# ghnmqdtg/VM-ASR

Hardware: AMD Instinct MI355X
Metric: audio clips/sec (train step) 48kHz n_fft=1024 (higher is better)
Workload: dtype bf16 (autocast over G; scan/STFT f32; MPD f32/bf16x3 MFMA); 1 GPU; vm_asr_48k_MPD.yaml full train step, DIMS 16 d_state 1 n_fft 1024 clip 122640@48k; per_gpu_batch=4, global_batch=4, parallelism=dp1, execution=hipGraph replay, 2 streams, generator_streams=2

## Files before the change

### include/vmasr_hip.h

```cpp
#ifndef VMASR_HIP_H
#define VMASR_HIP_H

#include <stddef.h>
#include <stdint.h>

#ifdef __cplusplus
extern "C" {
#endif

#define VMASR_ABI_VERSION 1

typedef void *vmasr_stream_t;

enum { VMASR_F32 = 0, VMASR_F16 = 1, VMASR_BF16 = 2 };

enum {
    VMASR_OK = 0,
    VMASR_EINVAL = -1,
    VMASR_EALIGN = -2,
    VMASR_ENOSPACE = -3
};

int vmasr_abi_version(void);
const char *vmasr_last_error(void);
// ... 181 lines not shown
    const float *bias;
    int64_t nseq;
    int32_t H;
    int32_t reserved;
} vmasr_cg_slot;
int vmasr_conv_mfma_supported(int32_t Cin, int32_t Cout, int32_t k, int32_t stride);
int vmasr_conv_mfma_supported_launch(int32_t Cin, int32_t Cout, int32_t k, int32_t stride, int32_t n, int64_t rows);
int vmasr_conv_mfma_config(int32_t pass, int32_t Cin, int32_t Cout, int32_t ops, int32_t out[3]);
void vmasr_conv_set_cu_limit(int32_t cus);
int32_t vmasr_conv_get_cu_limit(void);
int vmasr_conv_mfma_fwd(const vmasr_cg_slot *slots, int32_t n, int32_t Cin, int32_t Cout, int32_t k, int32_t stride, int32_t pad,
                        int64_t rows_out, int32_t act, vmasr_stream_t stream);
int vmasr_conv_mfma_dgrad(const vmasr_cg_slot *slots, int32_t n, int32_t Cin, int32_t Cout, int32_t k, int32_t stride, int32_t pad,
                          int64_t rows_in, vmasr_stream_t stream);
int vmasr_conv_f32_fwd(const vmasr_cg_slot *slots, int32_t n, int32_t Cin, int32_t Cout, int32_t k, int32_t stride, int32_t pad,
                       int64_t rows_out, int32_t act, vmasr_stream_t stream);
int vmasr_conv_f32_dgrad(const vmasr_cg_slot *slots, int32_t n, int32_t Cin, int32_t Cout, int32_t k, int32_t stride, int32_t pad,
                         int64_t rows_in, vmasr_stream_t stream);
int vmasr_conv_mfma_wgrad(const vmasr_cg_slot *slots, int32_t n, int32_t Cin, int32_t Cout, int32_t k, int32_t stride, int32_t pad,
                          int32_t splits, vmasr_stream_t stream);
typedef struct vmasr_cg_gelu_bwd {
    const float *pre;
    const signed char *sgn;
    int64_t valid;
    float scale;
    int32_t reserved;
    float *db;
} vmasr_cg_gelu_bwd;
int vmasr_conv_mfma_dgrad_gelu(const vmasr_cg_slot *slots, const vmasr_cg_gelu_bwd *epi, const float *gtok, int32_t n, int32_t Cin, int32_t Cout,
                               int32_t k, int32_t stride, int32_t pad, int64_t rows_in, vmasr_stream_t stream);

int vmasr_wgrad_finish_multi(const float *const *parts, float *const *dws, float *const *dbs, float *const *e1s, float *const *e2s,
                             const int32_t *Ss, const int32_t *Ns, const int32_t *Ks, const int32_t *lds, int32_t n, vmasr_stream_t stream);

int vmasr_linear_f64acc(const float *x, const float *w, const float *bias, float *y, int64_t rows, int32_t out_features,
                        int32_t in_features, vmasr_stream_t stream);

typedef struct vmasr_adamw_item {
    float *p;
    const float *g;
    float *m;
    float *v;
    void *lp;
    int64_t n;
    float weight_decay;
    int32_t vec;
    void *lpt;
    int32_t rows, cols;
} vmasr_adamw_item;
int32_t vmasr_adamw_chunk(void);
int vmasr_adamw_step(const vmasr_adamw_item *items, const int32_t *chunks, int32_t nchunks, int64_t total_elems, const float *lr,
                     const float *step, float beta1, float beta2, float eps, vmasr_stream_t stream);

typedef struct vmasr_grad_segment {
    const float *ptr;
    int64_t n;
} vmasr_grad_segment;
size_t vmasr_grad_norm_workspace(int32_t nchunks);
int vmasr_grad_norm(const vmasr_grad_segment *segments, const int32_t *chunks, int32_t nchunks, int64_t total_elems, float max_norm,
                    float *state, void *workspace, size_t ws_bytes, vmasr_stream_t stream);
int vmasr_adamw_step_guarded(const vmasr_adamw_item *items, const int32_t *chunks, int32_t nchunks, int64_t total_elems, const float *lr,
                             const float *step, float beta1, float beta2, float eps, const float *state, float *const *step_counters,
                             int32_t ncounters, vmasr_stream_t stream);

typedef struct vmasr_sgd_item {
    float *p;
// ... 221 lines not shown
    VMASR_K_BIAS_GELU,
    VMASR_K_SS2D_TRANSPOSE,
    VMASR_K_SS2D_FWD_AGG,
    VMASR_K_SS2D_CARRY,
    VMASR_K_SS2D_FWD_APPLY,
    VMASR_K_SS2D_MERGE,
    VMASR_K_SS2D_BWD_AGG,
    VMASR_K_SS2D_BWD_APPLY,
    VMASR_K_SS2D_PRE,
    VMASR_K_LN_GATE,
    VMASR_K_STACK_ROWS,
    VMASR_K_FEAT_L1,
    VMASR_K_ADAMW,
    VMASR_K_CONV_POST,
    VMASR_K_CONV_POST_BWD_GELU,
    VMASR_K_WEIGHT_T,
    VMASR_K_MLP_FWD,
    VMASR_K_MLP_BWD,
    VMASR_K_GMLP_FWD,
    VMASR_K_GMLP_BWD,
    VMASR_K_INPROJ_FWD,
    VMASR_K_INPROJ_BWD,
    VMASR_K_SS2D_DEEP_XPROJ,
    VMASR_K_SS2D_DEEP_FWD,
    VMASR_K_SS2D_DEEP_BWD,
    VMASR_K_SS2D_DEEP_XBWD,
    VMASR_K_OUTPROJ_FWD,
    VMASR_K_OUTPROJ_BWD,
    VMASR_K_STFT_LOSS,
    VMASR_K_CONV_MFMA_FWD,
    VMASR_K_CONV_MFMA_DGRAD,
    VMASR_K_CONV_MFMA_WGRAD,
    VMASR_K_WGRAD_FINISH,
    VMASR_K_SKINNY_LINEAR,
    VMASR_K_METRICS,
    VMASR_K_RESAMPLE_DESIGN,
    VMASR_K_DEGRADE_BATCH,
    VMASR_K_GCONV1D_FWD,
    VMASR_K_GCONV1D_DGRAD,
    VMASR_K_GCONV1D_WGRAD,
    VMASR_K_GCONV1D_WGRAD_REDUCE,
    VMASR_K_STEM1D_FWD,
    VMASR_K_STEM1D_BWD,
    VMASR_K_STEM1D_BWD_REDUCE,
    VMASR_K_DCONV1D_FWD,
    VMASR_K_DCONV1D_DGRAD,
    VMASR_K_DCONV1D_REDUCE,
    VMASR_K_DCONV1D_WGRAD,
    VMASR_K_DCONV1D_WGRAD_REDUCE,
    VMASR_K_GRAD_NORM,
    VMASR_K_SGD,
    VMASR_K_RESAMPLE,
    VMASR_K_COUNT
};
void vmasr_set_deterministic(int on);
int vmasr_get_deterministic(void);
int64_t vmasr_det_timeouts(void);
void vmasr_prof_enable(int on);
void vmasr_prof_reset(void);
const char *vmasr_prof_name(int kernel_id);
int vmasr_prof_collect(int kernel_id, int64_t *launches, double *total_ms, double *alg_bytes);
int vmasr_mark_time(uint64_t *dst, vmasr_stream_t stream);

int vmasr_im2col2d_rows(const void *x, void *cols, int32_t B, int32_t C, int32_t H, int32_t W, int32_t kh, int32_t kw, int32_t sh, int32_t sw,
                        int32_t ph, int32_t pw, const int64_t *x_strides, int32_t x_dtype, int32_t cols_dtype, vmasr_stream_t stream);
int vmasr_col2im2d_rows(const void *gcols, void *dx, int32_t B, int32_t C, int32_t H, int32_t W, int32_t kh, int32_t kw, int32_t sh, int32_t sw,
// ... 11 lines not shown
```

### vm_asr_amd/_lib.py

```python
import ctypes
import os

from . import knobs

_HERE = os.path.dirname(os.path.abspath(__file__))
LIB_PATH = knobs.get("VMASR_LIB") or os.path.join(_HERE, "libvmasr_hip.so")

c_i32, c_i64, c_vp, c_sz = ctypes.c_int32, ctypes.c_int64, ctypes.c_void_p, ctypes.c_size_t

F32, F16, BF16 = 0, 1, 2


class SScanParams(ctypes.Structure):
    _fields_ = (
        [(n, c_i32) for n in ("batch", "dim", "seqlen", "dstate", "n_groups", "n_chunks", "dtype",
                              "delta_softplus")]
        + [(n, c_i64) for n in ("A_d_stride", "A_dstate_stride",
                                "B_batch_stride", "B_group_stride", "B_dstate_stride",
                                "C_batch_stride", "C_group_stride", "C_dstate_stride",
                                "u_batch_stride", "u_d_stride", "delta_batch_stride", "delta_d_stride",
                                "out_batch_stride", "out_d_stride")]
        + [(n, c_vp) for n in ("A_ptr", "B_ptr", "C_ptr", "D_ptr", "u_ptr", "delta_ptr",
                               "delta_bias_ptr", "out_ptr", "x_ptr")]
    )
# ... 106 lines not shown
    "vmasr_adamw_step_guarded": (ctypes.c_int, [c_vp, c_vp, c_i32, c_i64, c_vp, c_vp, ctypes.c_float, ctypes.c_float, ctypes.c_float, c_vp, c_vp, c_i32, c_vp]),
    "vmasr_sgd_step": (ctypes.c_int, [c_vp, c_vp, c_i32, c_i64, c_vp, ctypes.c_float, c_i32, c_vp]),
    "vmasr_sgd_step_guarded": (ctypes.c_int, [c_vp, c_vp, c_i32, c_i64, c_vp, ctypes.c_float, c_i32, c_vp, c_vp]),
    "vmasr_grad_norm_workspace": (c_sz, [c_i32]),
    "vmasr_grad_norm": (ctypes.c_int, [c_vp, c_vp, c_i32, c_i64, ctypes.c_float, c_vp, c_vp, c_sz, c_vp]),
    "vmasr_masked_l1_blocks": (c_i32, []),
    "vmasr_masked_l1_fwd": (ctypes.c_int, [c_vp, c_vp, c_vp, c_vp, c_vp, c_vp, c_i32, c_i64, c_i64, c_i32, c_vp]),
    "vmasr_masked_l1_bwd": (ctypes.c_int, [c_vp, c_vp, c_vp, c_vp, c_vp, c_i32, c_i64, c_i32, c_vp]),
    "vmasr_lsgan_fwd": (ctypes.c_int, [c_vp, c_vp, c_vp, c_i32, c_vp, c_vp]),
    "vmasr_lsgan_bwd": (ctypes.c_int, [c_vp, c_vp, c_vp, c_vp, c_i32, c_vp, c_vp]),
    "vmasr_masked_l1_bwd_add": (ctypes.c_int, [c_vp, c_vp, c_vp, c_vp, c_vp, c_vp, c_i32, c_i64, c_i32, c_vp]),
    "vmasr_sum_parts": (ctypes.c_int, [c_vp, c_vp, c_i32, c_i32, c_i32, c_i64, c_vp]),
    "vmasr_weight_prep_split": (ctypes.c_int, [c_vp, c_vp, c_i32, c_i32, c_i32, c_vp]),
    "vmasr_weight_transpose": (ctypes.c_int, [c_vp, c_vp, c_vp, c_vp, c_i32, c_i32, c_i32, c_i32, c_vp]),
    "vmasr_gelu_bwd_split": (ctypes.c_int, [c_vp, c_vp, c_vp, c_vp, c_vp, c_vp, c_i32, c_i64, c_i32, c_vp]),
    "vmasr_conv_mfma_supported": (ctypes.c_int, [c_i32, c_i32, c_i32, c_i32]),
    "vmasr_conv_mfma_supported_launch": (ctypes.c_int, [c_i32, c_i32, c_i32, c_i32, c_i32, ctypes.c_int64]),
    "vmasr_conv_mfma_config": (ctypes.c_int, [c_i32, c_i32, c_i32, c_i32, ctypes.POINTER(c_i32)]),
    "vmasr_mark_time": (ctypes.c_int, [c_vp, c_vp]),
    "vmasr_im2col2d_rows": (ctypes.c_int, [c_vp, c_vp] + [c_i32] * 10 + [c_vp, c_i32, c_i32, c_vp]),
    "vmasr_col2im2d_rows": (ctypes.c_int, [c_vp, c_vp] + [c_i32] * 10 + [c_vp, c_i32, c_i32, c_vp]),
    "vmasr_skinny_linear_supported": (ctypes.c_int, [c_i64, c_i32, c_i32]),
    "vmasr_skinny_linear": (ctypes.c_int, [c_vp, c_vp, c_vp, c_vp, c_i64, c_i32, c_i32, c_i64, c_i64, c_i32, c_i32, c_vp]),
    "vmasr_conv_set_cu_limit": (None, [c_i32]),
    "vmasr_conv_get_cu_limit": (c_i32, []),
    "vmasr_conv_mfma_fwd": (ctypes.c_int, [ctypes.POINTER(CgSlot), c_i32, c_i32, c_i32, c_i32, c_i32, c_i32, c_i64, c_i32, c_vp]),
    "vmasr_conv_mfma_dgrad": (ctypes.c_int, [ctypes.POINTER(CgSlot), c_i32, c_i32, c_i32, c_i32, c_i32, c_i32, c_i64, c_vp]),
    "vmasr_conv_f32_fwd": (ctypes.c_int, [ctypes.POINTER(CgSlot), c_i32, c_i32, c_i32, c_i32, c_i32, c_i32, c_i64, c_i32, c_vp]),
    "vmasr_conv_f32_dgrad": (ctypes.c_int, [ctypes.POINTER(CgSlot), c_i32, c_i32, c_i32, c_i32, c_i32, c_i32, c_i64, c_vp]),
    "vmasr_conv_mfma_wgrad": (ctypes.c_int, [ctypes.POINTER(CgSlot), c_i32, c_i32, c_i32, c_i32, c_i32, c_i32, c_i32, c_vp]),
    "vmasr_conv_mfma_dgrad_gelu": (ctypes.c_int, [ctypes.POINTER(CgSlot), ctypes.POINTER(CgGeluBwd), c_vp, c_i32, c_i32, c_i32, c_i32, c_i32,
                                                  c_i32, c_i64, c_vp]),
    "vmasr_wgrad_finish_multi": (ctypes.c_int, [c_vp, c_vp, c_vp, c_vp, c_vp, c_vp, c_vp, c_vp, c_vp, c_i32, c_vp]),
    "vmasr_linear_f64acc": (ctypes.c_int, [c_vp, c_vp, c_vp, c_vp, c_i64, c_i32, c_i32, c_vp]),
    "vmasr_ss2d_glue_supported": (ctypes.c_int, [c_i32, c_i32, c_i32]),
    "vmasr_ss2d_pre_fwd": (ctypes.c_int, [c_vp, c_vp, c_vp, c_i32, c_i32, c_i32, c_i32, c_vp]),
    "vmasr_ss2d_pre_bwd": (ctypes.c_int, [c_vp, c_vp, c_vp, c_vp, c_i32, c_i32, c_i32, c_i32, c_vp]),
    "vmasr_ln_gate_fwd": (ctypes.c_int, [c_vp] * 7 + [c_i32, c_i32, c_i32, ctypes.c_float, c_i32, c_vp]),
    "vmasr_ln_gate_bwd": (ctypes.c_int, [c_vp] * 11 + [c_i32, c_i32, c_i32, c_i32, c_vp]),
    "vmasr_ln_gate_bwd_workspace": (c_i64, [c_i32, c_i32, c_i32, c_i32]),
    "vmasr_ln_gate_bwd_ws": (ctypes.c_int, [c_vp] * 12 + [c_i32, c_i32, c_i32, c_i32, c_vp]),
    "vmasr_ln_gate_pair_supported": (ctypes.c_int, [c_i32, c_i32, c_i32]),
    "vmasr_ln_gate_pair_fwd": (ctypes.c_int, [c_vp] * 8 + [c_i32, c_i32, c_i32, c_i32, ctypes.c_float, c_i32, c_vp]),
    "vmasr_ln_gate_pair_bwd": (ctypes.c_int, [c_vp] * 13 + [c_i32, c_i32, c_i32, c_i32, c_i32, c_vp]),
    "vmasr_ss2d_supported": (ctypes.c_int, [c_i32] * 5),
    "vmasr_ss2d_part_floats": (c_sz, [c_i32] * 4),
    "vmasr_ss2d_fwd": (ctypes.c_int, [ctypes.POINTER(SS2DParams), c_vp]),
    "vmasr_ss2d_bwd": (ctypes.c_int, [ctypes.POINTER(SS2DParams), c_vp]),
    "vmasr_ss2d_deep_supported": (ctypes.c_int, [c_i32] * 5),
    "vmasr_ss2d_deep_waves_per_row": (c_i32, [c_i32, c_i32]),
    "vmasr_ss2d_deep_fwd": (ctypes.c_int, [ctypes.POINTER(SS2DDeepParams), c_vp]),
    "vmasr_ss2d_deep_bwd": (ctypes.c_int, [ctypes.POINTER(SS2DDeepParams), c_vp]),
    "vmasr_set_deterministic": (None, [ctypes.c_int]),
    "vmasr_get_deterministic": (ctypes.c_int, []),
    "vmasr_det_timeouts": (ctypes.c_int64, []),
    "vmasr_prof_enable": (None, [ctypes.c_int]),
    "vmasr_prof_reset": (None, []),
    "vmasr_prof_name": (ctypes.c_char_p, [ctypes.c_int]),
    "vmasr_prof_collect": (ctypes.c_int, [ctypes.c_int, ctypes.POINTER(ctypes.c_int64),
                                          ctypes.POINTER(ctypes.c_double), ctypes.POINTER(ctypes.c_double)]),
    "vmasr_prof_collect_shapes": (ctypes.c_int, [ctypes.c_int, ctypes.c_int, ctypes.POINTER(ctypes.c_double), ctypes.POINTER(ctypes.c_int64),
                                                 ctypes.POINTER(ctypes.c_double)]),
    "vmasr_cross_scan": (ctypes.c_int, [c_vp, c_vp, c_i32, c_i32, c_i32, c_i32, c_i32, c_vp]),
    "vmasr_cross_merge": (ctypes.c_int, [c_vp, c_vp, c_i32, c_i32, c_i32, c_i32, c_i32, c_vp]),
    "vmasr_dwconv_silu_fwd": (ctypes.c_int, [c_vp, c_vp, c_vp, c_vp, c_i32, c_i32, c_i32, c_i32, c_i32, c_vp]),
    "vmasr_dwconv_silu_bwd": (ctypes.c_int, [c_vp, c_vp, c_vp, c_vp, c_vp, c_vp, c_vp, c_vp,
# ... 119 lines not shown
            conv[i] = ctypes.c_void_p(a.data_ptr())
        elif isinstance(a, ctypes.Structure):
            conv[i] = ctypes.byref(a)
    if device is None:
        raise RuntimeError(f"{what}: no tensor argument and no device= to launch on")
    with torch.cuda.device(device):
        check(fn(*conv, current_stream(device)), what)


def require_cuda(name, *tensors):
    if not all(t.is_cuda for t in tensors):
        raise RuntimeError(f"{name}: expected a CUDA (HIP) tensor; vm_asr_amd has no CPU path")


def bf16_autocast():
    import torch
    return torch.is_autocast_enabled("cuda") and torch.get_autocast_dtype("cuda") == torch.bfloat16


def autocast_dtype(x):
    import torch
    return torch.get_autocast_dtype("cuda") if torch.is_autocast_enabled("cuda") else x.dtype


def f32c(t, shape):
    return t.detach().float().reshape(shape).contiguous()


def rows2d(t, width):
    t2 = t.reshape(-1, width)
    return t2 if t2.is_contiguous() else t2.contiguous()


K_COUNT = 82


def zeros_f32(device, *shapes):
    import torch
    sizes = [0 if sh is None else -(-int(torch.Size(sh).numel()) // 4) * 4 for sh in shapes]
    flat = torch.zeros(max(1, sum(sizes)), dtype=torch.float32, device=device)
    out, off = [], 0
    for sh, n in zip(shapes, sizes):
        out.append(None if sh is None else flat[off:off + torch.Size(sh).numel()].view(sh))
        off += n
    return out


def prof_enable(on=True):
    lib().vmasr_prof_enable(int(bool(on)))


def prof_reset():
    lib().vmasr_prof_reset()


def prof_collect():
    l = lib()
    out = {}
    for k in range(K_COUNT):
        n, ms, by = ctypes.c_int64(0), ctypes.c_double(0.0), ctypes.c_double(0.0)
        check(l.vmasr_prof_collect(k, ctypes.byref(n), ctypes.byref(ms), ctypes.byref(by)), "prof_collect")
        if n.value:
            out[l.vmasr_prof_name(k).decode()] = dict(launches=n.value, ms=ms.value, alg_bytes=by.value)
    return out


def prof_collect_shapes(name, max_groups=16):
# ... 10 lines not shown
```

### vm_asr_amd/csrc/api.hip

```cpp
#include "common.h"

#include <mutex>
#include <vector>

namespace vmasr {
namespace {
thread_local char g_err[512] = "";

struct Rec {
    int kid;
    hipEvent_t e0, e1;
    double bytes;
};
std::mutex g_mu;
std::vector<Rec> g_recs;
std::vector<hipEvent_t> g_pool;
thread_local Rec g_open{-1, nullptr, nullptr, 0.0};

hipEvent_t take_event() {
    if (!g_pool.empty()) {
        hipEvent_t e = g_pool.back();
        g_pool.pop_back();
        return e;
    }
    hipEvent_t e = nullptr;
    (void)hipEventCreate(&e);
    return e;
}

const char *kNames[VMASR_K_COUNT] = {
    "sscan_fwd", "sscan_fwd_agg", "sscan_fwd_carry", "sscan_fwd_apply", "sscan_bwd", "sscan_bwd_agg",
    "sscan_bwd_carry", "sscan_bwd_apply", "cross_scan", "cross_merge", "dwconv_silu_fwd", "dwconv_silu_bwd_a",
    "dwconv_silu_bwd_b", "stft", "istft_frames", "istft_ola", "istft_bwd", "layer_norm_fwd", "layer_norm_bwd",
    "layer_norm_bwd_reduce", "small_linear_fwd", "small_linear_bwd", "small_linear_reduce",
    "xproj_fwd", "xproj_bwd_a", "xproj_bwd_b", "spectral_power_iter", "im2col_kx1", "col2im_kx1", "split_bf16", "bias_gelu",
    "ss2d_transpose", "ss2d_fwd_agg", "ss2d_carry", "ss2d_fwd_apply", "ss2d_merge", "ss2d_bwd_agg", "ss2d_bwd_apply",
    "ss2d_pre", "ln_gate", "stack_rows", "feat_l1", "adamw", "conv_post", "conv_post_bwd_gelu", "weight_transpose", "mlp_fwd", "mlp_bwd", "gmlp_fwd", "gmlp_bwd", "inproj_fwd", "inproj_bwd",
    "ss2d_deep_xproj", "ss2d_deep_fwd", "ss2d_deep_bwd", "ss2d_deep_xbwd", "outproj_fwd", "outproj_bwd", "stft_loss",
    "conv_mfma_fwd", "conv_mfma_dgrad", "conv_mfma_wgrad", "wgrad_finish", "skinny_linear", "metrics", "resample_design", "degrade_batch",
    "gconv1d_fwd", "gconv1d_dgrad", "gconv1d_wgrad", "gconv1d_wgrad_reduce",
    "stem1d_fwd", "stem1d_bwd", "stem1d_bwd_reduce",
    "dconv1d_fwd", "dconv1d_dgrad", "dconv1d_reduce", "dconv1d_wgrad", "dconv1d_wgrad_reduce", "grad_norm", "sgd", "resample_poly"};
}

bool g_prof_on = false;
static bool g_det_on = false;
constexpr int kMaxDev = 16;
static unsigned *g_det_buf[kMaxDev] = {};

unsigned *det_ticket(int kid) {
    if (!g_det_on || kid < 0 || kid >= VMASR_K_COUNT) return nullptr;
    int dev = 0;
    if (hipGetDevice(&dev) != hipSuccess || dev < 0 || dev >= kMaxDev || g_det_buf[dev] == nullptr) {
        set_error("deterministic mode: no ticket buffer for device %d (vmasr_set_deterministic(1) must run before the first launch)", dev);
        return nullptr;
    }
    return g_det_buf[dev] + kid;
}
static int det_prepare() {
    int n = 0, cur = 0;
    if (hipGetDeviceCount(&n) != hipSuccess || n <= 0) return 0;
    (void)hipGetDevice(&cur);
    int rc = 0;
    for (int d = 0; d < n && d < kMaxDev; ++d) {
        if (g_det_buf[d]) continue;
        if (hipSetDevice(d) != hipSuccess || hipMalloc(reinterpret_cast<void **>(&g_det_buf[d]), 2 * VMASR_K_COUNT * sizeof(unsigned)) != hipSuccess ||
            hipMemset(g_det_buf[d], 0, 2 * VMASR_K_COUNT * sizeof(unsigned)) != hipSuccess || hipDeviceSynchronize() != hipSuccess) {
            g_det_buf[d] = nullptr;
            set_error("deterministic mode: cannot allocate the ticket buffer of device %d (switch the mode on outside a stream capture)", d);
            rc = VMASR_EINVAL;
        }
    }
// ... 121 lines not shown
```

### vm_asr_amd/csrc/wgrad.hip

```cpp
#include <algorithm>

#include "common.h"

namespace vmasr {
namespace {

constexpr int kMaxWgItems = 40;
struct WgItem {
    const float *parts;
    float *dw;
    float *db;
    float *e1, *e2;
    int S, N, K, ld;
};
struct WgTable {
    WgItem it[kMaxWgItems];
};

__global__ __launch_bounds__(256) void wgrad_finish_multi_kernel(const WgTable t) {
    const WgItem &w = t.it[blockIdx.y];
    const int cols = w.K + (w.db ? 1 : 0) + (w.e1 ? 1 : 0) + (w.e2 ? 1 : 0);
    const long total = (long)w.N * cols;
    const size_t sstride = (size_t)w.N * w.ld;
    for (long i = (long)blockIdx.x * blockDim.x + threadIdx.x; i < total; i += (long)gridDim.x * blockDim.x) {
        const int n = (int)(i / cols), k = (int)(i - (long)n * cols);
        const float *p = w.parts + (size_t)n * w.ld + k;
        float s = 0.f;
        for (int j = 0; j < w.S; ++j) s += p[(size_t)j * sstride];
        if (k < w.K) w.dw[(size_t)n * w.K + k] = s;
        else if (k == w.K) w.db[n] = s;
        else if (k == w.K + 1) w.e1[n] = s;
        else w.e2[n] = s;
    }
}

}
}

using namespace vmasr;

VMASR_EXPORT int vmasr_wgrad_finish_multi(const float *const *parts, float *const *dws, float *const *dbs, float *const *e1s, float *const *e2s, const int32_t *Ss,
                                          const int32_t *Ns, const int32_t *Ks, const int32_t *lds, int32_t n, vmasr_stream_t stream) {
    VMASR_REQUIRE(parts && dws && dbs && Ss && Ns && Ks && lds && n > 0, VMASR_EINVAL, "wgrad_finish_multi: null argument");
    hipStream_t st = static_cast<hipStream_t>(stream);
    for (int j = 0; j < n; ++j) {
        const float *e1 = e1s ? e1s[j] : nullptr, *e2 = e2s ? e2s[j] : nullptr;
        VMASR_REQUIRE((!e1 || dbs[j]) && (!e2 || e1), VMASR_EINVAL, "wgrad_finish_multi: item %d: extra columns need the ones before them", j);
        VMASR_REQUIRE(parts[j] && dws[j] && Ss[j] > 0 && Ns[j] > 0 && Ks[j] > 0 && lds[j] >= Ks[j] + (dbs[j] ? 1 : 0) + (e1 ? 1 : 0) + (e2 ? 1 : 0), VMASR_EINVAL,
                      "wgrad_finish_multi: bad item %d", j);
    }
    for (int base = 0; base < n; base += kMaxWgItems) {
        const int m = std::min(kMaxWgItems, n - base);
        WgTable t{};
        long maxel = 0;
        double bytes = 0;
        for (int i = 0; i < m; ++i) {
            const int j = base + i;
            float *e1 = e1s ? e1s[j] : nullptr, *e2 = e2s ? e2s[j] : nullptr;
            t.it[i] = WgItem{parts[j], dws[j], dbs[j], e1, e2, Ss[j], Ns[j], Ks[j], lds[j]};
            maxel = std::max(maxel, (long)Ns[j] * (Ks[j] + 3));
            bytes += (double)Ss[j] * Ns[j] * lds[j] * 4 + (double)Ns[j] * (Ks[j] + 1) * 4;
        }
        const int gx = (int)std::min<long>(std::max<long>((maxel + 255) / 256, 1), 64);
        VMASR_LAUNCH(VMASR_K_WGRAD_FINISH, bytes, wgrad_finish_multi_kernel, dim3(gx, m), dim3(256), 0, st, t);
    }
    return check_launch("wgrad_finish_multi");
}
```

### vm_asr_amd/knobs.py

```python
import os
import warnings
from collections import namedtuple

Knob = namedtuple("Knob", "name kind default values reader doc parse")


def _bad(k, raw, allowed):
    return ValueError(f"{k.name}={raw!r}: expected {allowed}")


def _flag(k, raw):
    if raw == "1":
        return True
    if raw == "0":
        return False
    raise _bad(k, raw, "0 or 1")


def _choice(k, raw):
    if raw in k.values:
        return raw
    raise _bad(k, raw, "one of " + " | ".join(k.values))


# ... 88 lines not shown
    _k("VMASR_MPD_FUSE_GELU_BWD", "flag", 1, "the activation backward inside the input-gradient epilogue"),
    _k("VMASR_SN_STACK", "flag", 1, "spectral normalisation, stack and permutation of a layer's weights in one launch"),
    _k("VMASR_STACK_INPUT", "flag", 1, "a layer reads the previous layer's stacked output directly"),
    _k("VMASR_CONV_POST", "flag", 1, "the 1-channel output convolution straight on the stacked maps"),
    _k("VMASR_CONV_FIRST", "flag", 1, "the 1 -> 32 channel input convolution + GELU straight from the folded signals"),
    _k("VMASR_FEAT_TAP", "flag", 1, "a feature map's gradient (next layer's + feature-matching loss's) formed in one pass"),
    _k("VMASR_FEAT_L1", "flag", 1, "the feature-matching loss on the stacked maps in one kernel"),
    _k("VMASR_MSD_CONV", "choice", "hip", "the MSD's strided grouped 1-D convolutions: hip = the exact-fp32 MFMA kernels (csrc/gconv1d.hip), "
       "torch = F.conv1d (A/B measurements, double backward)", values=("hip", "torch"), reader="python:msd"),
    _k("VMASR_MSD_STEM", "choice", "hip", "the MSD's 1 -> hidden stem convolution + GELU: hip = one fused pass that keeps no pre-activation "
       "(csrc/stem1d.hip), torch = F.conv1d + F.gelu (A/B measurements, double backward)", values=("hip", "torch"), reader="python:msd"),
    _k("VMASR_MSD_FEAT", "choice", "hip", "the MSD's feature-matching loss in the generator's pass: hip = formed on the way (the stem's share inside "
       "the stem kernels, the other maps in the one-pass L1 kernel; msd_featmatch.py), torch = forward_single + the loop of sub, abs, mean",
       values=("hip", "torch"), reader="python:msd"),
    _k("VMASR_MSD_TAIL", "choice", "torch", "the MSD's dense tail (8h -> 8h k 5 + GELU, conv_post): hip = the exact-fp32 MFMA kernels with ordered "
       "split-K sums (csrc/dconv1d.hip: bit-identical run to run, no library algorithm search), torch = F.conv1d + F.gelu (the default: "
       "faster on the 8h -> 8h layer, profiles/msd_tail.md; double backward)", values=("hip", "torch"), reader="python:msd"),
    _k("VMASR_TWO_STREAM", "choice", "1", "the discriminator on a side stream: 1 on, 0 one stream, force also in deterministic mode (test hook)",
       values=("1", "0", "force")),
    _k("VMASR_SHARE_FAKE_PASS", "flag", 1, "one discriminator pass over the fake batch serves both phases of the step"),
    _k("VMASR_GEN_STREAMS", "choice", "auto", "the generator's phase branch on a stream of its own in captured steps: auto where the trainer says so, "
       "1 off, 2 on, 2eager on in eager steps too (debugging aid)", values=("auto", "1", "2", "2eager")),
    _k("VMASR_GEN_LANES", "list", None, "comma list of the segments that leave the main stream (pe,e0..e3,d0..d3,out,ia); unset = all (dev aid)",
       parse=_comma_list),
    _k("VMASR_STEP_VARIANT", "variant", None, "pins the captured step layout: one | lane | lane:<share of the CUs for the discriminator's backward>",
       values=("one", "lane", "lane:0.75"), parse=_step_variant),
    _k("VMASR_SIDE_CUS", "int", None, "CU limit of the discriminator's convolutions beside the generator's backward (and forward unless "
       "VMASR_SIDE_CUS_FWD is set); 0 = no limit; unset = Trainer.side_cu_limits()"),
    _k("VMASR_SIDE_CUS_FWD", "int", None, "the same beside the generator's forward"),
    _k("VMASR_SIDE_CUS_MINC", "int", 0, "the backward limit only for layers at least this wide"),
    _k("VMASR_GRAPH_GC_GUARD", "flag", 1, "no cyclic garbage collection between a graph capture and its first replays"),
    _k("VMASR_PHASE_EVENTS", "flag", 0, "device-clock marks at the step's phase boundaries (tools/phase_probe.py)"),
    _k("VMASR_LN_DEFER", "flag", 1, "LayerNorm's dgamma / dbeta of a whole backward pass reduced in one launch"),
    _k("VMASR_HIP_ADAMW", "flag", 1, "the multi-tensor AdamW kernel on the flat gradient buffers"),
    _k("VMASR_FUSED_ADAMW", "flag", 1, "torch's fused AdamW where the HIP kernel does not apply"),
    _k("VMASR_HIP_SGD", "flag", 1, "the multi-tensor SGD kernel on the flat gradient buffers (TRAIN.OPTIMIZER.NAME sgd; fused_sgd.py); 0 = "
       "optimizer.step(), which graph capture refuses", reader="python:sgd"),
    _k("VMASR_LP_SHADOWS", "flag", 1, "bf16 shadow copies of the parameters, refreshed by the optimiser kernel"),
    _k("VMASR_LP_SHADOWS_T", "flag", 1, "transposed bf16 shadows of the 2-D weights too"),
    _k("VMASR_RESUME_CONFIG_MISMATCH", "choice", "raise", "a checkpoint written under another configuration: raise or warn", values=("raise", "warn")),
    _k("VMASR_DIST_BACKEND", "str", None, "torch.distributed backend; unset = nccl on a GPU, else gloo"),
    _k("VMASR_DIST_TIMEOUT_S", "int", 600, "process-group timeout in seconds"),
    _k("VMASR_RCCL_TIMEOUT_S", "float", 300.0, "watchdog of a captured collective in seconds (rccl.py)"),
    _k("VMASR_RCCL_DIRECT", "flag", 0, "the trainer's own RCCL communicator outside captures too"),
    _k("VMASR_GRAPH_COLLECTIVES", "flag", 0, "capture the gradient all-reduces into the step's graph"),
    _k("VMASR_OVERLAP_REDUCE", "flag", 1, "asynchronous gradient all-reduces; 0 = strictly between the graphs"),
    _k("VMASR_GRAD_COMM", "choice", "fp32", "wire dtype of the gradient all-reduce: fp32, mpd-bf16 the discriminator's as bf16, bf16 both",
       values=("fp32", "mpd-bf16", "bf16")),
    _k("VMASR_GRAD_COMM_EMULATE", "choice", None, "one rank: the 16-bit wire's rounding applied to this rank's own gradient", values=("mpd-bf16", "bf16")),
    _csrc("VMASR_CONV_CU_SLACK", 24, "convgemm.hip: CUs by which the convolution CU limit is soft"),
    _csrc("VMASR_CONV_TILE", 0, "convgemm.hip: 128 forces the small tile"),
    _csrc("VMASR_CONV_MFMA", 16, "convgemm.hip: 16 = the 16x16x32 MFMA form, 32 = 32x32x16"),
    _csrc("VMASR_CONV_F32_TILE", 128, "convgemm.hip: tile of the exact-fp32 form, 128 or 256"),
    _csrc("VMASR_XPROJ_MFMA", 0, "xproj.hip: 1 = the MFMA kernels (measured slower)"),
    _csrc("VMASR_SSCAN_N_RB", 0, "sscan_n.hip: rows per workgroup; 0 = planned"),
    _csrc("VMASR_SSCAN_N_PP", 0, "sscan_n.hip: state pairs per wave; 0 = planned"),
    _csrc("VMASR_BWD_WAVES", 0, "sscan.hip: waves of the d_state-1 backward; 0 = 8"),
    _csrc("VMASR_SSCAN_N_LEGACY", 0, "sscan.hip: non-zero = the one-state-at-a-time kernels for general d_state (A/B)"),
    _external("VMASR_BENCH_WATCHDOG", "bench.py: seconds after which a wedged run dumps its stacks and exits"),
    _external("VMASR_PARITY_TABLE", "tests/conftest.py: path of the achieved-error table the session writes"),
    _external("VMASR_TEST_CLIPS", "tests/test_fullsize.py: clips of the full-size accuracy test"),
    _external("VMASR_ORACLE_LIB", "oracle/oracle.py: path of the oracle library (sanitizer build)"),
    _external("VMASR_REFERENCE", "tests/golden/_refload.py: checkout of the reference project that regenerates the goldens"),
)}


# ... 16 lines not shown
```

### vm_asr_amd/wgrad.py

```python
import numpy as np
import torch

from . import _lib
from . import layernorm as _ln
from .linear import _mm_acc, splitk_plan

__all__ = ["weight_grad_finished"]


class _Queue:
    def __init__(self):
        self.items = []

    def reset(self):
        self.items = []

    def flush(self):
        items, self.items = self.items, []
        if items:
            _launch(items)
            for it in items:
                for param, (st, ptr, shape) in ((it["wparam"], it["dw_ref"]), (it["bparam"], it["db_ref"])) + tuple(it.get("extra", ())):
                    if param is None or st is None or param.grad is None or param.grad.data_ptr() == ptr:
                        continue
                    param.grad.copy_(torch.empty(0, dtype=torch.float32, device=param.grad.device).set_(st, 0, shape).view_as(param.grad))


_Q = _Queue()
_ln._flush_hooks.append(_Q)


def _launch(items):
    n = len(items)
    arr = lambda k, dt: np.array([it[k] for it in items], dtype=dt)
    parts, dws, dbs = arr("parts_ptr", np.uint64), arr("dw_ptr", np.uint64), arr("db_ptr", np.uint64)
    e1s = np.array([it.get("e1_ptr", 0) for it in items], dtype=np.uint64)
    e2s = np.array([it.get("e2_ptr", 0) for it in items], dtype=np.uint64)
    Ss, Ns, Ks, lds = arr("S", np.int32), arr("N", np.int32), arr("K", np.int32), arr("ld", np.int32)
    _lib.call(_lib.lib().vmasr_wgrad_finish_multi, parts.ctypes.data, dws.ctypes.data, dbs.ctypes.data, e1s.ctypes.data, e2s.ctypes.data,
              Ss.ctypes.data, Ns.ctypes.data, Ks.ctypes.data, lds.ctypes.data, n, device=items[0]["parts"].device)


def _parts(gy2, x2):
    rows, out_f = gy2.shape
    in_f = x2.shape[1]
    S = splitk_plan(rows, out_f, in_f)
    if S < 4 or rows % S:
        return _mm_acc(gy2.t(), x2, torch.float32).unsqueeze(0)
    chunk = rows // S
    return _mm_acc(gy2.unflatten(0, (S, chunk)).transpose(1, 2), x2.unflatten(0, (S, chunk)), torch.float32)


def weight_grad_finished(gy2, x_aug, K, weight=None, bias=None, fresh=False):
    parts = _parts(gy2, x_aug).contiguous()
    S, N, ld = parts.shape
    has_b = ld > K
    dev = parts.device
    dw = torch.empty((N, K), dtype=torch.float32, device=dev)
    db = torch.empty(N, dtype=torch.float32, device=dev) if has_b else None
    ref = lambda t: (None, 0, None) if t is None else (t.untyped_storage(), t.data_ptr(), tuple(t.shape))
    item = dict(parts=parts, parts_ptr=parts.data_ptr(), dw_ptr=dw.data_ptr(), db_ptr=0 if db is None else db.data_ptr(), S=S, N=N, K=K,
                ld=ld, wparam=weight, bparam=bias, dw_ref=ref(dw), db_ref=ref(db))
    if _ln.DEFER_REDUCE and fresh and dev.type == "cuda":
        _ln.ensure_callback()
        _Q.items.append(item)
    else:
        _launch([item])
    return dw, db


def finish_slabs(parts, K, outs, params, fresh):
    S, N, ld = parts.shape
    dw, db, e1, e2 = (tuple(outs) + (None,) * 4)[:4]
    ref = lambda t: (None, 0, None) if t is None else (t.untyped_storage(), t.data_ptr(), tuple(t.shape))
    pw, pb, p1, p2 = (tuple(params) + (None,) * 4)[:4]
    item = dict(parts=parts, parts_ptr=parts.data_ptr(), dw_ptr=dw.data_ptr(), db_ptr=0 if db is None else db.data_ptr(),
                e1_ptr=0 if e1 is None else e1.data_ptr(), e2_ptr=0 if e2 is None else e2.data_ptr(), S=S, N=N, K=K, ld=ld,
                wparam=pw, bparam=pb, dw_ref=ref(dw), db_ref=ref(db), extra=((p1, ref(e1)), (p2, ref(e2))))
    if _ln.DEFER_REDUCE and fresh and parts.device.type == "cuda":
        _ln.ensure_callback()
        _Q.items.append(item)
    else:
        _launch([item])
```

Measured before the change: 199.5 clips/s.

## Batch bf16 weight-gradient GEMMs into one grouped MFMA launch at backward end

```diff
diff --git a/include/vmasr_hip.h b/include/vmasr_hip.h
--- a/include/vmasr_hip.h
+++ b/include/vmasr_hip.h
@@ -237,6 +237,13 @@
 
 int vmasr_wgrad_finish_multi(const float *const *parts, float *const *dws, float *const *dbs, float *const *e1s, float *const *e2s,
                              const int32_t *Ss, const int32_t *Ns, const int32_t *Ks, const int32_t *lds, int32_t n, vmasr_stream_t stream);
+
+int vmasr_wgrad_gemm_supported(int32_t N, int32_t ld, int32_t dtype);
+int32_t vmasr_wgrad_gemm_plan(int64_t rows, int32_t N, int32_t ld);
+int32_t vmasr_wgrad_gemm_chunk(int64_t rows, int32_t S);
+int vmasr_wgrad_gemm_multi(const void *const *gys, const void *const *xs, float *const *parts, const int32_t *rows, const int32_t *Ss,
+                           const int32_t *Ns, const int32_t *lds, const int32_t *ldgs, const int32_t *ldxs, int32_t dtype, int32_t n,
+                           vmasr_stream_t stream);
 
 int vmasr_linear_f64acc(const float *x, const float *w, const float *bias, float *y, int64_t rows, int32_t out_features,
                         int32_t in_features, vmasr_stream_t stream);
@@ -524,6 +531,7 @@
     VMASR_K_CONV_MFMA_DGRAD,
     VMASR_K_CONV_MFMA_WGRAD,
     VMASR_K_WGRAD_FINISH,
+    VMASR_K_WGRAD_GEMM,
     VMASR_K_SKINNY_LINEAR,
     VMASR_K_METRICS,
     VMASR_K_RESAMPLE_DESIGN,
diff --git a/vm_asr_amd/_lib.py b/vm_asr_amd/_lib.py
--- a/vm_asr_amd/_lib.py
+++ b/vm_asr_amd/_lib.py
@@ -162,6 +162,10 @@
     "vmasr_conv_mfma_dgrad_gelu": (ctypes.c_int, [ctypes.POINTER(CgSlot), ctypes.POINTER(CgGeluBwd), c_vp, c_i32, c_i32, c_i32, c_i32, c_i32,
                                                   c_i32, c_i64, c_vp]),
     "vmasr_wgrad_finish_multi": (ctypes.c_int, [c_vp, c_vp, c_vp, c_vp, c_vp, c_vp, c_vp, c_vp, c_vp, c_i32, c_vp]),
+    "vmasr_wgrad_gemm_supported": (ctypes.c_int, [c_i32, c_i32, c_i32]),
+    "vmasr_wgrad_gemm_plan": (c_i32, [c_i64, c_i32, c_i32]),
+    "vmasr_wgrad_gemm_chunk": (c_i32, [c_i64, c_i32]),
+    "vmasr_wgrad_gemm_multi": (ctypes.c_int, [c_vp] * 9 + [c_i32, c_i32, c_vp]),
     "vmasr_linear_f64acc": (ctypes.c_int, [c_vp, c_vp, c_vp, c_vp, c_i64, c_i32, c_i32, c_vp]),
     "vmasr_ss2d_glue_supported": (ctypes.c_int, [c_i32, c_i32, c_i32]),
     "vmasr_ss2d_pre_fwd": (ctypes.c_int, [c_vp, c_vp, c_vp, c_i32, c_i32, c_i32, c_i32, c_vp]),
@@ -347,7 +351,7 @@
     return t2 if t2.is_contiguous() else t2.contiguous()
 
 
-K_COUNT = 82
+K_COUNT = 83
 
 
 def zeros_f32(device, *shapes):
diff --git a/vm_asr_amd/csrc/api.hip b/vm_asr_amd/csrc/api.hip
--- a/vm_asr_amd/csrc/api.hip
+++ b/vm_asr_amd/csrc/api.hip
@@ -37,7 +37,7 @@
     "ss2d_transpose", "ss2d_fwd_agg", "ss2d_carry", "ss2d_fwd_apply", "ss2d_merge", "ss2d_bwd_agg", "ss2d_bwd_apply",
     "ss2d_pre", "ln_gate", "stack_rows", "feat_l1", "adamw", "conv_post", "conv_post_bwd_gelu", "weight_transpose", "mlp_fwd", "mlp_bwd", "gmlp_fwd", "gmlp_bwd", "inproj_fwd", "inproj_bwd",
     "ss2d_deep_xproj", "ss2d_deep_fwd", "ss2d_deep_bwd", "ss2d_deep_xbwd", "outproj_fwd", "outproj_bwd", "stft_loss",
-    "conv_mfma_fwd", "conv_mfma_dgrad", "conv_mfma_wgrad", "wgrad_finish", "skinny_linear", "metrics", "resample_design", "degrade_batch",
+    "conv_mfma_fwd", "conv_mfma_dgrad", "conv_mfma_wgrad", "wgrad_finish", "wgrad_gemm", "skinny_linear", "metrics", "resample_design", "degrade_batch",
     "gconv1d_fwd", "gconv1d_dgrad", "gconv1d_wgrad", "gconv1d_wgrad_reduce",
     "stem1d_fwd", "stem1d_bwd", "stem1d_bwd_reduce",
     "dconv1d_fwd", "dconv1d_dgrad", "dconv1d_reduce", "dconv1d_wgrad", "dconv1d_wgrad_reduce", "grad_norm", "sgd", "resample_poly"};
diff --git a/vm_asr_amd/csrc/wgrad.hip b/vm_asr_amd/csrc/wgrad.hip
--- a/vm_asr_amd/csrc/wgrad.hip
+++ b/vm_asr_amd/csrc/wgrad.hip
@@ -34,10 +34,203 @@
     }
 }
 
+typedef __bf16 bf16x8 __attribute__((ext_vector_type(8)));
+typedef __bf16 bf16x4 __attribute__((ext_vector_type(4)));
+typedef float f32x16 __attribute__((ext_vector_type(16)));
+typedef unsigned u32x4 __attribute__((ext_vector_type(4)));
+typedef __attribute__((address_space(3))) bf16x4 lds_bf16x4;
+
+constexpr int kGgMaxItems = 40;
+constexpr int kGgRows = 32;
+constexpr int kGgWaveTiles = 7;
+constexpr int kGgMaxTiles = 4 * kGgWaveTiles;
+constexpr int kGgMaxPanels = 12;
+constexpr int kGgPanelBytes = kGgRows * 64;
+constexpr int kGgStage = kGgMaxPanels * kGgPanelBytes;
+constexpr int kGgPasses = kGgMaxPanels / 2;
+constexpr int kGgMaxSlabs = 4096;
+
+struct GgItem {
+    const bf16_t *gy, *x;
+    float *parts;
+    int rows, S, N, ld, ldg, ldx, chunk, u0;
+};
+struct GgTable {
+    GgItem it[kGgMaxItems];
+    int n, units;
+};
+static_assert(sizeof(GgTable) <= 4096, "GgTable is passed by value as the kernel's argument block");
+
+__device__ __forceinline__ bf16x8 gg_frag(const unsigned char *panel, const int ks, const int lane_off) {
+    const unsigned char *p = panel + ks * (16 * 64) + lane_off;
+    const bf16x4 lo = __builtin_amdgcn_ds_read_tr16_b64_v4bf16((lds_bf16x4 *)p);
+    const bf16x4 hi = __builtin_amdgcn_ds_read_tr16_b64_v4bf16((lds_bf16x4 *)(p + 4 * 64));
+    return __builtin_shufflevector(lo, hi, 0, 1, 2, 3, 4, 5, 6, 7);
+}
+
+__global__ __launch_bounds__(256, 2) void wgrad_gemm_multi_kernel(const GgTable t) {
+    __shared__ __attribute__((aligned(16))) unsigned char smem[2 * kGgStage];
+    const int tid = threadIdx.x, lane = tid & 63, wave = __builtin_amdgcn_readfirstlane(tid >> 6);
+    const int lg = lane >> 4, lq = (lane & 15) >> 2, lp = lane & 3;
+    const int lane_off = (8 * (lg >> 1) + lq) * 64 + (2 * (lg & 1) + (lp >> 1)) * 16 + 8 * (lp & 1);
+    const u32x4 z4 = {0u, 0u, 0u, 0u};
+
+#pragma unroll 1
+    for (int u = blockIdx.x; u < t.units; u += gridDim.x) {
+        int i = 0;
+        while (i + 1 < t.n && u >= t.it[i + 1].u0) ++i;
+        const GgItem &w = t.it[i];
+        const int s = u - w.u0;
+        const int N = w.N, ld = w.ld;
+        const int TM = (N + 31) >> 5, TL = (ld + 31) >> 5, ntiles = TM * TL, npan = TM + TL;
+        const long rb = (long)s * w.chunk;
+        const int rbeg = (int)(rb < (long)w.rows ? rb : (long)w.rows);
+        const int rend = (int)(rb + w.chunk < (long)w.rows ? rb + w.chunk : (long)w.rows);
+        const int nk = (rend - rbeg + kGgRows - 1) / kGgRows;
+
+        const bf16_t *src[kGgPasses];
+        int srow[kGgPasses];
+        bool act[kGgPasses], colok[kGgPasses], isx[kGgPasses];
+#pragma unroll
+        for (int p = 0; p < kGgPasses; ++p) {
+            const int idx = tid + 256 * p, pan = idx >> 7, row = (idx >> 2) & 31, cl = idx & 3;
+            act[p] = pan < npan;
+            isx[p] = pan >= TM;
+            const int col = ((isx[p] ? pan - TM : pan) * 4 + cl) * 8;
+            colok[p] = act[p] && col < (isx[p] ? ld : N);
+            srow[p] = rbeg + row;
+            src[p] = (isx[p] ? w.x + (size_t)srow[p] * w.ldx : w.gy + (size_t)srow[p] * w.ldg) + col;
+        }
+        const size_t step_g = (size_t)kGgRows * w.ldg, step_x = (size_t)kGgRows * w.ldx;
+        u32x4 reg[kGgPasses];
+
+        int pa[kGgWaveTiles], pb[kGgWaveTiles];
+        f32x16 acc[kGgWaveTiles];
+#pragma unroll
+        for (int k = 0; k < kGgWaveTiles; ++k) {
+            const int tt = wave + 4 * k, ti = tt / TL, tj = tt - ti * TL;
+            pa[k] = ti * kGgPanelBytes;
+            pb[k] = (TM + tj) * kGgPanelBytes;
+#pragma unroll
+            for (int r = 0; r < 16; ++r) acc[k][r] = 0.f;
+        }
+
+#define GG_LOAD()                                                                                   \
+    do {                                                                                            \
+        _Pragma("unroll") for (int p = 0; p < kGgPasses; ++p) {                                     \
+            reg[p] = z4;                                                                            \
+            if (colok[p] && srow[p] < rend) reg[p] = *reinterpret_cast<const u32x4 *>(src[p]);      \
+            src[p] += isx[p] ? step_x : step_g;                                                     \
+            srow[p] += kGgRows;                                                                     \
+        }                                                                                           \
+    } while (0)
+#define GG_STORE(buf)                                                                               \
+    do {                                                                                            \
+        _Pragma("unroll") for (int p = 0; p < kGgPasses; ++p)                                       \
+            if (act[p]) *reinterpret_cast<u32x4 *>(smem + (buf) * kGgStage + (tid + 256 * p) * 16) = reg[p]; \
+    } while (0)
+
+        if (nk > 0) {
+            GG_LOAD();
+            GG_STORE(0);
+        }
+        __syncthreads();
+        for (int kt = 0; kt < nk; ++kt) {
+            const int buf = kt & 1;
+            const bool more = kt + 1 < nk;
+            if (more) GG_LOAD();
+            const unsigned char *st = smem + buf * kGgStage;
+#pragma unroll
+            for (int ks = 0; ks < 2; ++ks)
+#pragma unroll
+                for (int k = 0; k < kGgWaveTiles; ++k)
+                    if (wave + 4 * k < ntiles) {
+                        const bf16x8 a = gg_frag(st + pa[k], ks, lane_off);
+                        const bf16x8 b = gg_frag(st + pb[k], ks, lane_off);
+                        acc[k] = __builtin_amdgcn_mfma_f32_32x32x16_bf16(a, b, acc[k], 0, 0, 0);
+                    }
+            if (more) GG_STORE(buf ^ 1);
+            __syncthreads();
+        }
+#undef GG_LOAD
+#undef GG_STORE
+
+        float *out = w.parts + (size_t)s * N * ld;
+#pragma unroll
+        for (int k = 0; k < kGgWaveTiles; ++k) {
+            const int tt = wave + 4 * k;
+            if (tt < ntiles) {
+                const int ti = tt / TL, tj = tt - ti * TL;
+                const int col = tj * 32 + (lane & 31);
+#pragma unroll
+                for (int r = 0; r < 16; ++r) {
+                    const int row = ti * 32 + (r & 3) + 8 * (r >> 2) + 4 * (lane >> 5);
+                    if (row < N && col < ld) out[(size_t)row * ld + col] = acc[k][r];
+                }
+            }
+        }
+    }
+}
+
+bool gg_supported(int N, int ld, int dtype) {
+    if (dtype != VMASR_BF16 || N <= 0 || ld <= 0 || N % 8 || ld % 8) return false;
+    const int TM = (N + 31) / 32, TL = (ld + 31) / 32;
+    return TM * TL <= kGgMaxTiles && TM + TL <= kGgMaxPanels;
+}
+
+int gg_chunk(int64_t rows, int S) {
+    const int64_t per = (rows + S - 1) / S;
+    return (int)((per + kGgRows - 1) / kGgRows * kGgRows);
+}
+
 }
 }
 
 using namespace vmasr;
+
+VMASR_EXPORT int vmasr_wgrad_gemm_supported(int32_t N, int32_t ld, int32_t dtype) { return gg_supported(N, ld, dtype) ? 1 : 0; }
+
+VMASR_EXPORT int32_t vmasr_wgrad_gemm_plan(int64_t rows, int32_t N, int32_t ld) {
+    (void)N;
+    (void)ld;
+    if (rows <= 0) return 0;
+    const int S0 = (int)std::min<int64_t>(std::max<int64_t>(rows / 512, 1), 128);
+    const int64_t chunk = gg_chunk(rows, S0);
+    return (int32_t)((rows + chunk - 1) / chunk);
+}
+
+VMASR_EXPORT int32_t vmasr_wgrad_gemm_chunk(int64_t rows, int32_t S) { return (rows > 0 && S > 0) ? gg_chunk(rows, S) : 0; }
+
+VMASR_EXPORT int vmasr_wgrad_gemm_multi(const void *const *gys, const void *const *xs, float *const *parts, const int32_t *rows, const int32_t *Ss,
+                                        const int32_t *Ns, const int32_t *lds, const int32_t *ldgs, const int32_t *ldxs, int32_t dtype, int32_t n,
+                                        vmasr_stream_t stream) {
+    VMASR_REQUIRE(gys && xs && parts && rows && Ss && Ns && lds && ldgs && ldxs && n > 0, VMASR_EINVAL, "wgrad_gemm_multi: null argument");
+    hipStream_t st = static_cast<hipStream_t>(stream);
+    for (int j = 0; j < n; ++j) {
+        VMASR_REQUIRE(gg_supported(Ns[j], lds[j], dtype), VMASR_EINVAL, "wgrad_gemm_multi: item %d: (N %d, ld %d, dtype %d) is not supported", j, Ns[j],
+                      lds[j], dtype);
+        VMASR_REQUIRE(gys[j] && xs[j] && parts[j] && aligned_to(gys[j], 16) && aligned_to(xs[j], 16) && aligned_to(parts[j], 4) && rows[j] > 0 && Ss[j] > 0 &&
+                          Ss[j] <= kGgMaxSlabs && ldgs[j] >= Ns[j] && ldxs[j] >= lds[j] && ldgs[j] % 8 == 0 && ldxs[j] % 8 == 0,
+                      VMASR_EINVAL, "wgrad_gemm_multi: bad item %d", j);
+    }
+    for (int base = 0; base < n; base += kGgMaxItems) {
+        const int m = std::min(kGgMaxItems, n - base);
+        GgTable t{};
+        double bytes = 0;
+        int units = 0;
+        for (int i = 0; i < m; ++i) {
+            const int j = base + i;
+            t.it[i] = GgItem{static_cast<const bf16_t *>(gys[j]), static_cast<const bf16_t *>(xs[j]), parts[j], rows[j], Ss[j], Ns[j], lds[j], ldgs[j], ldxs[j],
+                             gg_chunk(rows[j], Ss[j]), units};
+            units += Ss[j];
+            bytes += (double)rows[j] * (Ns[j] + lds[j]) * 2 + (double)Ss[j] * Ns[j] * lds[j] * 4;
+        }
+        t.n = m;
+        t.units = units;
+        VMASR_LAUNCH(VMASR_K_WGRAD_GEMM, bytes, wgrad_gemm_multi_kernel, dim3(units), dim3(256), 0, st, t);
+    }
+    return check_launch("wgrad_gemm_multi");
+}
 
 VMASR_EXPORT int vmasr_wgrad_finish_multi(const float *const *parts, float *const *dws, float *const *dbs, float *const *e1s, float *const *e2s, const int32_t *Ss,
                                           const int32_t *Ns, const int32_t *Ks, const int32_t *lds, int32_t n, vmasr_stream_t stream) {
diff --git a/vm_asr_amd/knobs.py b/vm_asr_amd/knobs.py
--- a/vm_asr_amd/knobs.py
+++ b/vm_asr_amd/knobs.py
@@ -144,6 +144,8 @@
     _k("VMASR_GRAPH_GC_GUARD", "flag", 1, "no cyclic garbage collection between a graph capture and its first replays"),
     _k("VMASR_PHASE_EVENTS", "flag", 0, "device-clock marks at the step's phase boundaries (tools/phase_probe.py)"),
     _k("VMASR_LN_DEFER", "flag", 1, "LayerNorm's dgamma / dbeta of a whole backward pass reduced in one launch"),
+    _k("VMASR_WGRAD_GROUPED", "flag", 1, "the bf16 weight-gradient GEMMs of the fused VSS-block operators as one grouped MFMA launch at the end of "
+       "the backward pass (wgrad.py, csrc/wgrad.hip); 0 = one library GEMM each inside the block's backward", reader="python:wgrad"),
     _k("VMASR_HIP_ADAMW", "flag", 1, "the multi-tensor AdamW kernel on the flat gradient buffers"),
     _k("VMASR_FUSED_ADAMW", "flag", 1, "torch's fused AdamW where the HIP kernel does not apply"),
     _k("VMASR_HIP_SGD", "flag", 1, "the multi-tensor SGD kernel on the flat gradient buffers (TRAIN.OPTIMIZER.NAME sgd; fused_sgd.py); 0 = "
diff --git a/vm_asr_amd/wgrad.py b/vm_asr_amd/wgrad.py
--- a/vm_asr_amd/wgrad.py
+++ b/vm_asr_amd/wgrad.py
@@ -1,7 +1,7 @@
 import numpy as np
 import torch
 
-from . import _lib
+from . import _lib, knobs
 from . import layernorm as _ln
 from .linear import _mm_acc, splitk_plan
 
@@ -18,6 +18,7 @@
     def flush(self):
         items, self.items = self.items, []
         if items:
+            _launch_gemms(items)
             _launch(items)
             for it in items:
                 for param, (st, ptr, shape) in ((it["wparam"], it["dw_ref"]), (it["bparam"], it["db_ref"])) + tuple(it.get("extra", ())):
@@ -41,6 +42,29 @@
               Ss.ctypes.data, Ns.ctypes.data, Ks.ctypes.data, lds.ctypes.data, n, device=items[0]["parts"].device)
 
 
+def _launch_gemms(items):
+    gemms = [it for it in items if it.get("gemm") is not None]
+    if not gemms:
+        return
+    ops = [it.pop("gemm") for it in gemms]
+    arr = lambda vals, dt: np.array(vals, dtype=dt)
+    gys, xs = arr([g.data_ptr() for g, _ in ops], np.uint64), arr([x.data_ptr() for _, x in ops], np.uint64)
+    parts = arr([it["parts_ptr"] for it in gemms], np.uint64)
+    rows, ldgs, ldxs = (arr(v, np.int32) for v in ([g.shape[0] for g, _ in ops], [g.stride(0) for g, _ in ops], [x.stride(0) for _, x in ops]))
+    Ss, Ns, lds = (arr([it[k] for it in gemms], np.int32) for k in ("S", "N", "ld"))
+    _lib.call(_lib.lib().vmasr_wgrad_gemm_multi, gys.ctypes.data, xs.ctypes.data, parts.ctypes.data, rows.ctypes.data, Ss.ctypes.data,
+              Ns.ctypes.data, lds.ctypes.data, ldgs.ctypes.data, ldxs.ctypes.data, _lib.BF16, len(gemms), device=gemms[0]["parts"].device)
+
+
+def _grouped(gy2, x_aug):
+    if not (knobs.get("VMASR_WGRAD_GROUPED") and gy2.is_cuda and gy2.dtype == x_aug.dtype == torch.bfloat16 and gy2.dim() == x_aug.dim() == 2
+            and gy2.shape[0] == x_aug.shape[0] > 0 and gy2.stride(1) == x_aug.stride(1) == 1):
+        return False
+    if gy2.stride(0) % 8 or x_aug.stride(0) % 8 or gy2.data_ptr() % 16 or x_aug.data_ptr() % 16 or gy2.shape[0] >= 2 ** 31:
+        return False
+    return bool(_lib.lib().vmasr_wgrad_gemm_supported(gy2.shape[1], x_aug.shape[1], _lib.BF16))
+
+
 def _parts(gy2, x2):
     rows, out_f = gy2.shape
     in_f = x2.shape[1]
@@ -52,7 +76,14 @@
 
 
 def weight_grad_finished(gy2, x_aug, K, weight=None, bias=None, fresh=False):
-    parts = _parts(gy2, x_aug).contiguous()
+    gemm = None
+    if _grouped(gy2, x_aug):
+        rows, N, ld = gy2.shape[0], gy2.shape[1], x_aug.shape[1]
+        S = _lib.lib().vmasr_wgrad_gemm_plan(rows, N, ld)
+        parts = torch.empty((S, N, ld), dtype=torch.float32, device=gy2.device)
+        gemm = (gy2, x_aug)
+    else:
+        parts = _parts(gy2, x_aug).contiguous()
     S, N, ld = parts.shape
     has_b = ld > K
     dev = parts.device
@@ -60,11 +91,12 @@
     db = torch.empty(N, dtype=torch.float32, device=dev) if has_b else None
     ref = lambda t: (None, 0, None) if t is None else (t.untyped_storage(), t.data_ptr(), tuple(t.shape))
     item = dict(parts=parts, parts_ptr=parts.data_ptr(), dw_ptr=dw.data_ptr(), db_ptr=0 if db is None else db.data_ptr(), S=S, N=N, K=K,
-                ld=ld, wparam=weight, bparam=bias, dw_ref=ref(dw), db_ref=ref(db))
+                ld=ld, wparam=weight, bparam=bias, dw_ref=ref(dw), db_ref=ref(db), gemm=gemm)
     if _ln.DEFER_REDUCE and fresh and dev.type == "cuda":
         _ln.ensure_callback()
         _Q.items.append(item)
     else:
+        _launch_gemms([item])
         _launch([item])
     return dw, db
 
```

After: 200.7 clips/s (median of 6 runs). About the same (+0.6%).
